# thoglu/jammy_flows

Hardware: AMD Instinct MI355X
Metric: log-prob evals/sec (batch 2^20), e4+s2+e4 / gggg+f+gggg (higher is better)
Workload: dtype f32; 1 GPU; pdf("e4+s2+e4","gggg+f+gggg") log-prob, unconditional pdf with autoregressive conditioning, 1048576 rows in total, row-sharded; batch_per_gpu=1048576, total_rows=1048576, parallelism=rows sharded over 1 GPU(s)

## Files before the change

### jammy_flows_amd/csrc/jf_cond_mchain.h

```cpp
#pragma once
#include <type_traits>

#include "jf_cond_split.h"
#include "jf_manifold.h"
#include "jf_mfma.h"

namespace jf {

constexpr int CM_HMAX = 128, CM_K1MAX = 28, CM_NMAX = 64;

template <typename T, typename CLayer, int NL = JF_MAX_MCHAIN> struct CmArgs {
    const T* in; int64_t in_stride;
    const T* W1; int64_t w1s; const T* b1;
    const T* W2; int64_t w2s; const T* b2;
    int K1, H, N;
    const T* x; int64_t xs;
    const T* ld_in;
    int64_t B;
    int n_layers, dim, tile_stride, scratch, tab;
    int col0[NL];
    CLayer L[NL];
    T* x_out; int64_t xos;
    T* ld_out;
    const T* blp_in; T* blp_out;
    int32_t* status;
};

template <typename T, class Fam, int NT, bool FWD, class Args>
__device__ __forceinline__ void cond_mchain_body(const Args& a, const int block, const int n_blocks, unsigned char* smem_raw) {
    using MF = Mfma16<T>;
    constexpr int MT = 16, KS = 4, NREG = 4, JH = CM_HMAX / MT;
    const int k1p = (a.K1 + KS - 1) / KS * KS, ldk = k1p + 1;
    const int np = (a.N + MT - 1) / MT * MT;
    constexpr int LDW = CM_HMAX + 1;
    T* W1s = reinterpret_cast<T*>(smem_raw);
    T* b1s = W1s + CM_HMAX * ldk;
    T* W2s = b1s + CM_HMAX;
    T* b2s = W2s + np * LDW;
    T* Xs = b2s + np + 8;
    T* tiles = Xs + NT * ldk;
    T* tabs = tiles + NT * a.tile_stride;
    const int tid = threadIdx.x, lane = tid & 63, wave = tid >> 6;
    const int li = lane & 15, lq = lane >> 4;
    const int64_t last = a.B - 1;
    for (int i = tid; i < CM_HMAX * k1p; i += NT) {
        const int r = i / k1p, c = i - r * k1p;
        W1s[r * ldk + c] = (r < a.H && c < a.K1) ? a.W1[(int64_t)r * a.w1s + c] : T(0);
    }
    for (int i = tid; i < CM_HMAX; i += NT) b1s[i] = i < a.H ? a.b1[i] : T(0);
    float w2_inv = 1.f;
    if constexpr (std::is_same<T, float>::value) {
        float amax = 0.f;
        for (int i = tid; i < a.N * a.H; i += NT) {
            const int r = i / a.H, c = i - r * a.H;
            amax = fmaxf(amax, fabsf(a.W2[(int64_t)r * a.w2s + c]));
        }
#pragma unroll
        for (int m = 32; m >= 1; m >>= 1) amax = fmaxf(amax, __shfl_xor(amax, m));
        float* red = reinterpret_cast<float*>(b2s + np);
        if (lane == 0) red[wave] = amax;
        __syncthreads();
        amax = red[0];
        for (int w = 1; w < NT / 64; ++w) amax = fmaxf(amax, red[w]);
        const int e = (amax > 0.f && amax < INFINITY) ? 14 - ilogbf(amax) : 0;
        const float wscale = ldexpf(1.0f, e);
        w2_inv = ldexpf(1.0f, -(e + 14));
        unsigned char* W2p = reinterpret_cast<unsigned char*>(W2s);
        for (int f = tid; f < (np / MT) * CS_KSTEPS * 64; f += NT) {
            const int fl = f & 63, s = (f >> 6) % CS_KSTEPS, ct = (f >> 6) / CS_KSTEPS;
            const int m = fl & 15, q = fl >> 4, col = ct * MT + m;
            f16x8 hi, lo;
#pragma unroll
            for (int i = 0; i < 8; ++i) {
                const int k = 16 * (2 * s + (i >> 2)) + 4 * q + (i & 3);
                const float w = (col < a.N && k < a.H) ? a.W2[(int64_t)col * a.w2s + k] * wscale : 0.f;
                const _Float16 h16 = (_Float16)w;
                hi[i] = h16; lo[i] = (_Float16)(w - (float)h16);
            }
            *reinterpret_cast<f16x8*>(W2p + (size_t)((ct * CS_KSTEPS + s) * 2 + 0) * CS_FRAG + fl * 16) = hi;
            *reinterpret_cast<f16x8*>(W2p + (size_t)((ct * CS_KSTEPS + s) * 2 + 1) * CS_FRAG + fl * 16) = lo;
        }
    } else {
        for (int i = tid; i < np * CM_HMAX; i += NT) {
            const int r = i / CM_HMAX, c = i - r * CM_HMAX;
            W2s[r * LDW + c] = (r < a.N && c < a.H) ? a.W2[(int64_t)r * a.w2s + c] : T(0);
        }
    }
    for (int i = tid; i < np; i += NT) b2s[i] = (i < a.N && a.b2) ? a.b2[i] : T(0);
    for (int64_t row0 = (int64_t)block * NT; row0 < a.B; row0 += (int64_t)n_blocks * NT) {
    __syncthreads();
    for (int i = tid; i < NT * k1p; i += NT) {
        const int r = i / k1p, c = i - r * k1p;
        const int64_t gr = row0 + r;
        Xs[r * ldk + c] = c < a.K1 ? a.in[(gr <= last ? gr : last) * a.in_stride + c] : T(0);
    }
    __syncthreads();

    T* tile = tiles + wave * 64 * a.tile_stride;
    for (int rt = 0; rt < 4; ++rt) {
        T hreg[JH][NREG];
        {
            typename MF::Acc acc[JH];
#pragma unroll
            for (int j = 0; j < JH; ++j)
#pragma unroll
                for (int r = 0; r < NREG; ++r) acc[j][r] = T(0);
            for (int s = 0; s < k1p / KS; ++s) {
                const int kk = s * KS + lq;
                const T xb = Xs[(wave * 64 + rt * MT + li) * ldk + kk];
#pragma unroll
                for (int j = 0; j < JH; ++j) acc[j] = MF::mma(W1s[(j * MT + li) * ldk + kk], xb, acc[j]);
            }
#pragma unroll
            for (int j = 0; j < JH; ++j)
#pragma unroll
                for (int r = 0; r < NREG; ++r) hreg[j][r] = M<T>::tanh_fast(acc[j][r] + b1s[j * MT + MF::row_of(r, lane)]);
        }
        if constexpr (std::is_same<T, float>::value) {
            f16x8 hH[CS_KSTEPS], hL[CS_KSTEPS];
#pragma unroll
            for (int s = 0; s < CS_KSTEPS; ++s) {
                using u32x4 = __attribute__((ext_vector_type(4))) unsigned;
                u32x4 q0, q1;
#pragma unroll
                for (int i = 0; i < 8; i += 2) {
                    const int j = 2 * s + (i >> 2), r = i & 3;
                    unsigned ph, pl;
                    cs_split16(hreg[j][r] * CS_H_SCALE, hreg[j][r + 1] * CS_H_SCALE, ph, pl);
                    q0[i >> 1] = ph; q1[i >> 1] = pl;
                }
                hH[s] = __builtin_bit_cast(f16x8, q0); hL[s] = __builtin_bit_cast(f16x8, q1);
            }
            const unsigned char* W2p = reinterpret_cast<const unsigned char*>(W2s);
            for (int ct = 0; ct < np / MT; ++ct) {
                f32x4 acc = {0.f, 0.f, 0.f, 0.f};
#pragma unroll
                for (int s = 0; s < CS_KSTEPS; ++s) {
                    const f16x8 aH = *reinterpret_cast<const f16x8*>(W2p + (size_t)((ct * CS_KSTEPS + s) * 2 + 0) * CS_FRAG + lane * 16);
                    const f16x8 aL = *reinterpret_cast<const f16x8*>(W2p + (size_t)((ct * CS_KSTEPS + s) * 2 + 1) * CS_FRAG + lane * 16);
                    acc = __builtin_amdgcn_mfma_f32_16x16x32_f16(aL, hH[s], acc, 0, 0, 0);
                    acc = __builtin_amdgcn_mfma_f32_16x16x32_f16(aH, hL[s], acc, 0, 0, 0);
                    acc = __builtin_amdgcn_mfma_f32_16x16x32_f16(aH, hH[s], acc, 0, 0, 0);
                }
#pragma unroll
                for (int v = 0; v < 4; ++v) {
                    const int c = ct * MT + 4 * lq + v;
                    tile[(rt * MT + li) * a.tile_stride + c] = acc[v] * w2_inv + b2s[c];
                }
            }
        } else
        for (int ct = 0; ct < np / MT; ++ct) {
            typename MF::Acc acc;
#pragma unroll
            for (int r = 0; r < NREG; ++r) acc[r] = T(0);
            const T* wrow = W2s + (ct * MT + li) * LDW;
#pragma unroll
            for (int j = 0; j < JH; ++j)
#pragma unroll
                for (int r = 0; r < NREG; ++r) acc = MF::mma(wrow[j * MT + MF::row_of(r, lane)], hreg[j][r], acc);
#pragma unroll
            for (int v = 0; v < NREG; ++v) {
                const int c = ct * MT + MF::row_of(v, lane);
                tile[(rt * MT + li) * a.tile_stride + c] = acc[v] + b2s[c];
            }
        }
    }
    __syncthreads();

    const int64_t row = row0 + tid;
    const bool active = row <= last;
    const int64_t rrow = active ? row : last;
    T x[3] = {T(0), T(0), T(0)};
#pragma unroll
    for (int d = 0; d < Fam::DIM; ++d) if (d < a.dim) x[d] = a.x[rrow * a.xs + d];
    T ld = a.ld_in ? a.ld_in[rrow] : T(0);
    LaneCtx<T> ctx;
    ctx.tab = tabs + tid * (a.tab + a.scratch);
    ctx.corr = ctx.tab + a.tab;
    ctx.bins = nullptr; ctx.bin_i = 0;
    ctx.oob = ctx.nonconv = ctx.nonfinite = false;
    ctx.lane_valid = active;
    const T* prow = tiles + tid * a.tile_stride;
    for (int i = 0; i < a.n_layers; ++i) {
        const int l = FWD ? i : a.n_layers - 1 - i;
        Fam::template apply<T, FWD>(a.L[l], prow + a.col0[l], x, ld, ctx);
    }
    bool bad = !M<T>::finite(ld);
#pragma unroll
    for (int d = 0; d < Fam::DIM; ++d) bad = bad || !M<T>::finite(x[d]);
    if (active) {
#pragma unroll
        for (int d = 0; d < Fam::DIM; ++d) if (d < a.dim) a.x_out[row * a.xos + d] = x[d];
        a.ld_out[row] = ld;
        if (a.blp_out) {
            T s = a.blp_in ? a.blp_in[row] : T(0);
#pragma unroll
            for (int d = 0; d < Fam::DIM; ++d) if (d < a.dim) s += T(-0.5) * x[d] * x[d] - M<T>::HALF_LN_2PI;
            a.blp_out[row] = s;
        }
    }
    status_add(a.status, JF_STATUS_NONFINITE, active && (bad || ctx.nonfinite));
    status_add(a.status, JF_STATUS_OUT_OF_RANGE, active && ctx.oob);
    status_add(a.status, JF_STATUS_NONCONVERGED, active && ctx.nonconv);
    }
}

}
```

### jammy_flows_amd/csrc/jf_manifold.h

```cpp
#pragma once
#include "jf_sphere.h"
#include "jf_spline.h"

namespace jf {

constexpr int JF_CORR_SCRATCH = 81;

template <typename T> struct LaneCtx {
    T* tab;
    T* corr;
    int64_t* bins;
    int bin_i;
    bool oob, nonconv, nonfinite;
    bool lane_valid;
    bool tab_built = false;
    __device__ __forceinline__ void put_bin(int b) {
        if (bins) bins[bin_i] = (int64_t)b;
        ++bin_i;
    }
};

template <typename T> __device__ __forceinline__ SplineDev<T> to_dev(const jf_spline_opts& s) {
    SplineDev<T> o;
    o.nb = s.num_bins; o.smooth = s.smooth; o.fix_first = s.fix_first; o.fix_second = s.fix_second; o.independent = s.independent;
    o.fix_bd = s.fix_bd; o.n_w = s.n_w; o.n_h = s.n_h; o.n_d = s.n_d;
    o.fix_bd_value = (T)s.fix_bd_value; o.min_w = (T)s.min_w; o.min_h = (T)s.min_h; o.min_d = (T)s.min_d; o.ratio = (T)s.ratio;
    return o;
}
__host__ __device__ inline int spline_row_len(const jf_spline_opts& s) { return s.n_w + s.n_h + s.n_d; }

__host__ inline bool sane_hh(int hh) { return hh >= JF_ROT_QUATERNION && hh <= 64; }
__host__ inline bool sane_spline(const jf_spline_opts& s) {
    return s.num_bins >= 1 && s.num_bins <= JF_SPLINE_CAP && s.n_w >= 0 && s.n_w <= 4 * JF_SPLINE_CAP && s.n_h >= 0 &&
           s.n_h <= 4 * JF_SPLINE_CAP && s.n_d >= 0 && s.n_d <= 4 * JF_SPLINE_CAP;
}

template <class Fam, class = void> struct fam_tab_words { static int of(const typename Fam::CLayer&) { return JF_SPLINE_TAB; } };
template <class Fam> struct fam_tab_words<Fam, std::void_t<decltype(&Fam::tab_words)>> { static int of(const typename Fam::CLayer& L) { return Fam::tab_words(L); } };

template <typename T> __device__ __forceinline__ T r_core(const jf_r_layer& L, const T* __restrict__ p, T x, T& ld, LaneCtx<T>& c, bool inverse) {
    x = x > T(1) ? T(1) : (x < T(-1) ? T(-1) : x);
    bool oob;
    const SplineDev<T> o = to_dev<T>(L.sp);
    const SplineOut<T> r = spline_interval<T>(p, o, c.tab, x, inverse, (T)L.lo, (T)L.hi, oob, c.tab_built);
    c.oob = c.oob || oob;
    c.put_bin(r.bin);
    ld += r.lad;
    return r.y > T(1) ? T(1) : (r.y < T(-1) ? T(-1) : r.y);
}
struct RFam {
    using CLayer = jf_r_layer;
    static constexpr int DIM = 1;
    static constexpr bool HAS_BUILD = true;
    template <typename T> static __device__ __forceinline__ void build(const CLayer& L, const T* __restrict__ p, T* __restrict__ tab) {
        spline_interval_build<T>(p, to_dev<T>(L.sp), tab, (T)L.lo, (T)L.hi);
    }
    static __host__ bool sane(const CLayer& L) { return sane_spline(L.sp); }
    static __host__ int row_len(const CLayer& L) { return spline_row_len(L.sp); }
    static __host__ int n_bins(const CLayer&) { return 1; }
    static __host__ bool needs_tab(const CLayer&) { return true; }
    static __host__ int tab_words(const CLayer& L) { return spline_tab_words(L.sp.num_bins); }
    template <typename T, bool FWD> static __device__ __forceinline__ void apply(const CLayer& L, const T* __restrict__ p, T (&x)[3], T& ld, LaneCtx<T>& c) {
        if constexpr (FWD) {
            if (L.first) x[0] = real_line_to_interval<T>(x[0], (T)L.lo, (T)L.hi, ld);
            x[0] = r_core<T>(L, p, x[0], ld, c, false);
        } else {
            x[0] = r_core<T>(L, p, x[0], ld, c, true);
            if (L.first) x[0] = interval_to_real_line<T>(x[0], (T)L.lo, (T)L.hi, ld);
        }
    }
};

template <typename T> __device__ __forceinline__ T s1_rotate(const T* __restrict__ vs, int hh, T phi, bool transpose) {
    T e[3];
    s1_to_eucl<T>(phi, e);
    rotate_embed<T, 2>(vs, hh, e, transpose);
    return eucl_to_s1<T>(e);
}

template <typename T> __device__ __forceinline__ void s2_rotate(const T* __restrict__ vs, int hh, T (&x)[3], T& ld, bool transpose) {
    T e[3];
    s2_to_eucl<T>(x[0], x[1], e, ld);
    rotate_embed<T, 3>(vs, hh, e, transpose);
// ... 228 lines not shown
        }
    }
    static __host__ bool sane(const CLayer& L) {
        if (!sane_hh(L.hh_iter) || L.n_vertical < 0 || L.n_vertical > JF_MAX_NESTED || L.n_circular < 0 || L.n_circular > JF_MAX_NESTED) return false;
        if (L.corr_hidden < 0 || L.corr_hidden > 65536 || L.corr_rank < 0 || L.corr_rank > 65536) return false;
        for (int i = 0; i < L.n_vertical; ++i) if (!sane_spline(L.vertical[i].sp)) return false;
        for (int i = 0; i < L.n_circular; ++i) if (!sane_spline(L.circular[i].sp) || !sane_hh(L.circular[i].hh_iter)) return false;
        return true;
    }
    static __host__ int row_len(const CLayer& L) {
        int n = rot_len(L.hh_iter, 3) + n_kappa(L);
        for (int i = 0; i < L.n_vertical; ++i) n += spline_row_len(L.vertical[i].sp);
        if (L.correlated) return n + corr_len(L);
        for (int i = 0; i < L.n_circular; ++i) n += spline_row_len(L.circular[i].sp);
        return n;
    }
    static __host__ int n_bins(const CLayer& L) { return L.n_vertical + L.n_circular; }
    static __host__ bool needs_tab(const CLayer& L) { return L.n_vertical + L.n_circular > 0; }
    static __host__ int tab_words(const CLayer& L) {
        int w = 1;
        for (int i = 0; i < L.n_vertical && i < JF_MAX_NESTED; ++i) { const int t = spline_tab_words(L.vertical[i].sp.num_bins); w = t > w ? t : w; }
        for (int i = 0; i < L.n_circular && i < JF_MAX_NESTED; ++i) { const int t = spline_tab_words(L.circular[i].sp.num_bins); w = t > w ? t : w; }
        return w;
    }
    static __host__ int scratch(const CLayer& L) { return L.correlated ? JF_CORR_SCRATCH : 0; }

    template <typename T> static __device__ inline void corr_mlp(const CLayer& L, const T* __restrict__ mp, T z, T* __restrict__ out) {
        const int H = L.corr_hidden, R = L.corr_rank, n = corr_out(L);
        const T* W1 = mp;
        const T* b1 = mp + H;
        const T* s2 = mp + 2 * H;
        if (L.corr_full2) {
            const T* b2 = s2 + n * H;
            for (int i = 0; i < n; ++i) out[i] = b2[i];
            for (int j = 0; j < H; ++j) {
                const T h = M<T>::tanh(W1[j] * z + b1[j]);
                for (int i = 0; i < n; ++i) out[i] += s2[i * H + j] * h;
            }
        } else {
            const T* V = s2 + n * R;
            const T* b2 = V + R * H;
            T* t = out + n;
            for (int r = 0; r < R; ++r) t[r] = T(0);
            for (int j = 0; j < H; ++j) {
                const T h = M<T>::tanh(W1[j] * z + b1[j]);
                for (int r = 0; r < R; ++r) t[r] += V[r * H + j] * h;
            }
            for (int i = 0; i < n; ++i) {
                T acc = T(0);
                for (int r = 0; r < R; ++r) acc += s2[i * R + r] * t[r];
                out[i] = acc + b2[i];
            }
        }
    }

    template <typename T> static __device__ __forceinline__ void inv_head(const CLayer& L, const T* __restrict__ p, T (&x)[3], T& ld, T& ret_out, T& angle_out) {
        const T* fp = p + rot_len(L.hh_iter, 3);
        const T zs = (T)L.z_sign;
        const T kappa = kappa_of<T>(L, p, fp);
        if (L.hh_iter != 0) s2_rotate<T>(p, L.hh_iter, x, ld, true);
        const T prev = M<T>::cos(x[0]);
        ld += M<T>::log(M<T>::sin(safe_angle_pi<T>(x[0])));
        const T e2k = M<T>::exp(T(-2) * kappa);
        const T safe = kappa < T(100) ? M<T>::log(M<T>::expm1(T(2) * kappa)) : T(2) * kappa;
        ld += M<T>::log(T(2) * kappa) + kappa * (zs * prev + T(1)) - safe;
        T ret = zs * ((T(1) + e2k - T(2) * M<T>::exp(kappa * (zs * prev - T(1)))) / (T(-1) + e2k));
        if (kappa < M<T>::KAPPA_ID) ret = prev;
        ret = safe_cos<T>(ret, M<T>::EPS_COS);
        T angle = x[1];
        if (L.extra_rotation) inbetween<T>(ret, angle, ld, true);
        ret_out = ret; angle_out = angle;
    }
    template <typename T> static __device__ __forceinline__ void inv_tail(const CLayer& L, T ret, T angle, T (&x)[3], T& ld) {
        ret = safe_cos<T>(ret, M<T>::EPS_COS);
        const T th = M<T>::acos(ret);
        ld -= M<T>::log(M<T>::sin(safe_angle_pi<T>(th)));
        if (L.first) {
            T pl[3];
            s2_to_plane<T>(th, angle, pl, ld);
            x[0] = pl[0]; x[1] = pl[1];
        } else { x[0] = th; x[1] = angle; }
    }

    template <typename T, bool FWD> static __device__ __forceinline__ void apply(const CLayer& L, const T* __restrict__ p, T (&x)[3], T& ld, LaneCtx<T>& c) {
        const T* fp = p + rot_len(L.hh_iter, 3);
        const T zs = (T)L.z_sign, region = (T)L.identity_region;
        const T kappa = kappa_of<T>(L, p, fp);
        int nv = 0;
        for (int i = 0; i < L.n_vertical; ++i) nv += spline_row_len(L.vertical[i].sp);
        const T* vert = fp + n_kappa(L);
        const T* circ = vert + nv;
        if constexpr (!FWD) {
            T ret, angle;
            inv_head<T>(L, p, x, ld, ret, angle);
            const bool inside = (region == T(0)) || ((ret > T(-1) + region) && (ret < T(1) - region));
            if (L.correlated) {
                if (inside) {
                    const T z_in = ret;
                    int off = nv;
                    for (int i = L.n_vertical - 1; i >= 0; --i) {
                        off -= spline_row_len(L.vertical[i].sp);
                        ret = r_core<T>(L.vertical[i], vert + off, ret, ld, c, true);
                    }
                    corr_mlp<T>(L, vert + nv, z_in, c.corr);
                    int coff = corr_out(L);
                    for (int i = L.n_circular - 1; i >= 0; --i) {
                        coff -= rot_len(L.circular[i].hh_iter, 2) + spline_row_len(L.circular[i].sp);
                        T xx[3] = {angle, T(0), T(0)};
                        OFam::apply<T, false>(L.circular[i], c.corr + coff, xx, ld, c);
                        angle = xx[0];
                    }
                } else {
                    for (int i = 0; i < L.n_vertical + L.n_circular; ++i) c.put_bin(-2);
                }
            } else {
            if (L.n_circular > 0) {
                const T sc = azimuthal_scaling<T>(ret);
                int off = 0;
                for (int i = 0; i < L.n_circular; ++i) off += spline_row_len(L.circular[i].sp);
                for (int i = L.n_circular - 1; i >= 0; --i) {
                    off -= spline_row_len(L.circular[i].sp);
                    if (inside) angle = o_core<T>(L.circular[i], circ + off, angle, ld, c, false, sc);
                    else c.put_bin(-2);
                }
            }
            if (L.n_vertical > 0) {
                int off = nv;
                for (int i = L.n_vertical - 1; i >= 0; --i) {
                    off -= spline_row_len(L.vertical[i].sp);
                    if (inside) ret = r_core<T>(L.vertical[i], vert + off, ret, ld, c, true);
                    else c.put_bin(-2);
                }
            }
            }
            inv_tail<T>(L, ret, angle, x, ld);
        } else {
            if (L.first) {
                T pl[3] = {x[0], x[1], T(0)};
                plane_to_s2<T>(pl, x[0], x[1], ld);
            }
            T prev = M<T>::cos(x[0]);
            ld += M<T>::log(M<T>::sin(safe_angle_pi<T>(x[0])));
            T angle = x[1];
            const bool inside = (region == T(0)) || ((prev > T(-1) + region) && (prev < T(1) - region));
            if (L.correlated) {
                if (inside) {
                    int off = 0;
                    for (int i = 0; i < L.n_vertical; ++i) {
                        prev = r_core<T>(L.vertical[i], vert + off, prev, ld, c, false);
                        off += spline_row_len(L.vertical[i].sp);
                    }
                    corr_mlp<T>(L, vert + nv, prev, c.corr);
                    int coff = 0;
                    for (int i = 0; i < L.n_circular; ++i) {
                        T xx[3] = {angle, T(0), T(0)};
                        OFam::apply<T, true>(L.circular[i], c.corr + coff, xx, ld, c);
                        angle = xx[0];
                        coff += rot_len(L.circular[i].hh_iter, 2) + spline_row_len(L.circular[i].sp);
                    }
                } else {
                    for (int i = 0; i < L.n_vertical + L.n_circular; ++i) c.put_bin(-2);
                }
            } else {
            if (L.n_vertical > 0) {
                int off = 0;
                for (int i = 0; i < L.n_vertical; ++i) {
                    if (inside) prev = r_core<T>(L.vertical[i], vert + off, prev, ld, c, false);
                    else c.put_bin(-2);
                    off += spline_row_len(L.vertical[i].sp);
                }
            }
            if (L.n_circular > 0) {
                const T sc = azimuthal_scaling<T>(prev);
                int off = 0;
                for (int i = 0; i < L.n_circular; ++i) {
                    if (inside) angle = o_core<T>(L.circular[i], circ + off, angle, ld, c, true, sc);
                    else c.put_bin(-2);
                    off += spline_row_len(L.circular[i].sp);
                }
            }
            }
            if (L.extra_rotation) inbetween<T>(prev, angle, ld, false);
            ld -= M<T>::log(kappa * zs * prev + kappa / M<T>::tanh(kappa));
            T ret = zs * (T(1) + (T(1) / kappa) * M<T>::log(T(0.5) * (T(1) + zs * prev) + (T(0.5) - T(0.5) * zs * prev) * M<T>::exp(T(-2) * kappa)));
            if (kappa < M<T>::KAPPA_ID) ret = prev;
            ret = safe_cos<T>(ret, M<T>::EPS_COS);
            x[0] = M<T>::acos(ret);
            ld -= M<T>::log(M<T>::sin(safe_angle_pi<T>(x[0])));
            x[1] = angle;
            if (L.hh_iter != 0) s2_rotate<T>(p, L.hh_iter, x, ld, false);
        }
    }
};

}
```

### jammy_flows_amd/csrc/jf_math.h

```cpp
#pragma once
#include <hip/hip_runtime.h>
#include <math.h>

#include "jf_tanh_table.h"

namespace jf {

template <typename T> struct M;

template <typename T> struct DualTraits { static constexpr bool is_dual = false; using value_type = T; };
template <typename D> struct DualValues;



template <> struct M<float> {
    static constexpr float PI = 3.14159265358979323846f;
    static constexpr float TWO_PI = 6.28318530717958647692f;
    static constexpr float HALF_LN_2PI = 0.91893853320467274178f;
    static constexpr float SQRT2 = 1.41421356237309504880f;
    static constexpr float TINY = 1e-35f;
    static constexpr float EPS_COS = 1e-7f;
    static constexpr float EPS_S1 = 1e-5f;
    static constexpr float KAPPA_ID = 1e-4f;
#ifdef JF_PROBE_ACCURATE_EXP
    static __device__ __forceinline__ float exp_fast(float x) { return expf(x); }
#else
    static __device__ __forceinline__ float exp_fast(float x) { return __expf(x); }
#endif
#ifdef JF_PROBE_ACCURATE_LOG
    static __device__ __forceinline__ float log_fast(float x) { return logf(x); }
#else
    static __device__ __forceinline__ float log_fast(float x) { return 0.69314718056f * __builtin_amdgcn_logf(x); }
#endif
#ifdef JF_PROBE_ACCURATE_RCP
    static __device__ __forceinline__ float sqrt_fast(float x) { return sqrtf(x); }
    static __device__ __forceinline__ float rcp(float x) { return __fdiv_rn(1.0f, x); }
#else
    static __device__ __forceinline__ float sqrt_fast(float x) { return __builtin_amdgcn_sqrtf(x); }
    static __device__ __forceinline__ float rcp(float x) { return __builtin_amdgcn_rcpf(x); }
#endif
    static __device__ __forceinline__ float exp(float x) { return expf(x); }
    static __device__ __forceinline__ float log(float x) { return logf(x); }
    static __device__ __forceinline__ float log1p(float x) { return log1pf(x); }
    static __device__ __forceinline__ float expm1(float x) { return expm1f(x); }
    static __device__ __forceinline__ float sqrt(float x) { return sqrtf(x); }
    static __device__ __forceinline__ float erf(float x) { return erff(x); }
    static __device__ __forceinline__ float erfinv(float x) { return erfinvf(x); }
    static __device__ __forceinline__ float erfcinv(float x) { return erfcinvf(x); }
    static __device__ __forceinline__ float sin(float x) { return sinf(x); }
    static __device__ __forceinline__ float cos(float x) { return cosf(x); }
    static __device__ __forceinline__ float acos(float x) { return acosf(x); }
    static __device__ __forceinline__ float atan2(float y, float x) { return atan2f(y, x); }
    static __device__ __forceinline__ float tanh(float x) { return tanhf(x); }
    static __device__ __forceinline__ float tanh_fast(float x) { return 1.0f - 2.0f * __builtin_amdgcn_rcpf(__expf(2.0f * x) + 1.0f); }
    static __device__ __forceinline__ float abs(float x) { return fabsf(x); }
    static __device__ __forceinline__ float max(float a, float b) { return fmaxf(a, b); }
    static __device__ __forceinline__ float min(float a, float b) { return fminf(a, b); }
    static __device__ __forceinline__ bool finite(float x) { return isfinite(x); }
};

template <> struct M<double> {
    static constexpr double PI = 3.14159265358979323846;
    static constexpr double TWO_PI = 6.28318530717958647692;
    static constexpr double HALF_LN_2PI = 0.91893853320467274178;
    static constexpr double SQRT2 = 1.41421356237309504880;
    static constexpr double TINY = 1e-280;
    static constexpr double EPS_COS = 1e-10;
    static constexpr double EPS_S1 = 1e-8;
    static constexpr double KAPPA_ID = 1e-8;
    static __device__ __forceinline__ double exp_fast(double x) { return ::exp(x); }
    static __device__ __forceinline__ double log_fast(double x) {
        int e = __builtin_amdgcn_frexp_exp(x);
        double m = __builtin_amdgcn_frexp_mant(x);
        const bool low = m < 0.70710678118654752440;
        m = low ? m + m : m;
        e = low ? e - 1 : e;
        const double f = m - 1.0;
        const double s = f * rcp(2.0 + f);
        const double z = s * s, w = z * z;
        const double t1 = w * ::fma(w, ::fma(w, 1.531383769920937332e-01, 2.222219843214978396e-01), 3.999999999940941908e-01);
        const double t2 = z * ::fma(w, ::fma(w, ::fma(w, 1.479819860511658591e-01, 1.818357216161805012e-01), 2.857142874366239149e-01),
                                    6.666666666666735130e-01);
        const double R = t1 + t2, hfsq = 0.5 * f * f, de = (double)e;
        double r = ::fma(de, 6.93147180369123816490e-01, -((hfsq - ::fma(s, hfsq + R, de * 1.90821492927058770002e-10)) - f));
        r = x == 0.0 ? -INFINITY : r;
        return (x > 0.0 && x < INFINITY) || x == 0.0 ? r : (x < 0.0 ? NAN : x);
    }
    static __device__ __forceinline__ double sqrt_fast(double x) { return ::sqrt(x); }
    static __device__ __forceinline__ double rcp(double x) {
        const double r0 = __builtin_amdgcn_rcp(x);
        double r = ::fma(::fma(-x, r0, 1.0), r0, r0);
        r = ::fma(::fma(-x, r, 1.0), r, r);
        return isfinite(r) ? r : r0;
    }
    static __device__ __forceinline__ double exp(double x) { return ::exp(x); }
    static __device__ __forceinline__ double log(double x) { return ::log(x); }
    static __device__ __forceinline__ double log1p(double x) { return ::log1p(x); }
    static __device__ __forceinline__ double expm1(double x) { return ::expm1(x); }
    static __device__ __forceinline__ double sqrt(double x) { return ::sqrt(x); }
    static __device__ __forceinline__ double erf(double x) { return ::erf(x); }
    static __device__ __forceinline__ double erfinv(double x) { return ::erfinv(x); }
    static __device__ __forceinline__ double erfcinv(double x) { return ::erfcinv(x); }
    static __device__ __forceinline__ double sin(double x) { return ::sin(x); }
    static __device__ __forceinline__ double cos(double x) { return ::cos(x); }
    static __device__ __forceinline__ double acos(double x) { return ::acos(x); }
    static __device__ __forceinline__ double atan2(double y, double x) { return ::atan2(y, x); }
    static __device__ __forceinline__ double tanh(double x) { return ::tanh(x); }
    static __device__ __forceinline__ double tanh_fast(double x) {
        const double t = ::exp(-2.0 * ::fabs(x));
        return ::copysign((1.0 - t) * rcp(1.0 + t), x);
    }
    static __device__ __forceinline__ double abs(double x) { return ::fabs(x); }
    static __device__ __forceinline__ double max(double a, double b) { return ::fmax(a, b); }
    static __device__ __forceinline__ double min(double a, double b) { return ::fmin(a, b); }
    static __device__ __forceinline__ bool finite(double x) { return isfinite(x); }
};

__device__ __forceinline__ void tanh_tab_load(double* __restrict__ lds_tab, int tid, int nthreads) {
    for (int i = tid; i < JF_TANH_TAB_N; i += nthreads) lds_tab[i] = JF_TANH_TAB[i];
}
__device__ __forceinline__ double tanh_tab(const double* __restrict__ lds_tab, double x) {
#ifdef JF_PROBE_NO_TANH_TAB
    return M<double>::tanh_fast(x);
// ... 41 lines not shown
```

### jammy_flows_amd/csrc/manifold_kernels.hip

```cpp
#include <type_traits>

#include "jf_expmap.h"
#include "jf_manifold.h"

namespace jf {

constexpr int MC_MAX_PRE = 4;
template <typename T, typename CLayer> struct MChainArgs {
    const T* x; int64_t xs;
    const T* ld_in;
    const T* params; int64_t ps;
    int bcast;
    int64_t B;
    int n_layers;
    int dim;
    int tile_stride;
    int scratch;
    int tab;
    int rows;
    int shared_tab;
    int vec_ok[JF_MAX_MCHAIN];
    int col0[JF_MAX_MCHAIN];
    int ncols[JF_MAX_MCHAIN];
    CLayer L[JF_MAX_MCHAIN];
    T* x_out; int64_t xos;
    T* ld_out;
    const T* blp_in; T* blp_out;
    int64_t* bins; int64_t bins_stride;
    int32_t* status;
    const T* ld_pre[MC_MAX_PRE]; const T* blp_pre[MC_MAX_PRE];
    int n_ld_pre, n_blp_pre;
    T* total;
};

template <class Fam, class = void> struct fam_has_build : std::false_type {};
template <class Fam> struct fam_has_build<Fam, std::void_t<decltype(Fam::HAS_BUILD)>> : std::true_type {};

template <typename T, class Fam, bool FWD>
__global__ void __launch_bounds__(64) mchain_kernel(const MChainArgs<T, typename Fam::CLayer> a) {
    extern __shared__ __align__(16) unsigned char smem_raw[];
    T* tile = reinterpret_cast<T*>(smem_raw);
    const int tid = threadIdx.x;
    const int rows = a.rows;
    const int tile_rows = a.bcast ? 1 : rows;
    const bool lane_in = tid < rows;
    const int slot = lane_in ? tid : 0;
    constexpr bool CAN_SHARE = fam_has_build<Fam>::value;
    const bool shared = CAN_SHARE && a.shared_tab != 0;
    T* tab = tile + tile_rows * a.tile_stride + (shared ? 0 : slot * a.tab);
    const int64_t row0 = (int64_t)blockIdx.x * rows;
    const int64_t row = row0 + tid;
    const bool active = lane_in && row < a.B;
    const int64_t rrow = active ? row : a.B - 1;
    const int valid_rows = (int)((a.B - row0) < rows ? (a.B - row0) : rows);

    T x[3] = {T(0), T(0), T(0)};
#pragma unroll
    for (int d = 0; d < Fam::DIM; ++d) if (d < a.dim) x[d] = a.x[rrow * a.xs + d];
    T ld = a.ld_in ? a.ld_in[rrow] : T(0);
    LaneCtx<T> ctx;
    ctx.tab = tab;
    ctx.corr = tile + tile_rows * a.tile_stride + (shared ? 1 : rows) * a.tab + slot * a.scratch;
    ctx.bins = (a.bins && active) ? a.bins + row * a.bins_stride : nullptr;
    ctx.bin_i = 0;
    ctx.oob = ctx.nonconv = ctx.nonfinite = false;
    ctx.lane_valid = active;

    for (int i = 0; i < a.n_layers; ++i) {
        const int l = FWD ? i : a.n_layers - 1 - i;
        __syncthreads();
        if (a.bcast) {
            for (int j = tid; j < a.ncols[l]; j += 64) tile[j] = a.params[a.col0[l] + j];
        } else {
            stage_rows<T>(tile, a.tile_stride, a.params + row0 * a.ps + a.col0[l], a.ps, a.ncols[l], rows, valid_rows, tid, 64, a.vec_ok[l] != 0);
        }
        __syncthreads();
        const T* prow = tile + (a.bcast ? 0 : slot * a.tile_stride);
        if constexpr (CAN_SHARE) {
            if (shared) {
                if (tid == 0) Fam::template build<T>(a.L[l], prow, tab);
                __syncthreads();
                ctx.tab_built = true;
            }
        }
        if (lane_in) Fam::template apply<T, FWD>(a.L[l], prow, x, ld, ctx);
    }
    bool bad = !M<T>::finite(ld);
#pragma unroll
    for (int d = 0; d < Fam::DIM; ++d) bad = bad || !M<T>::finite(x[d]);
    if (active) {
#pragma unroll
        for (int d = 0; d < Fam::DIM; ++d) if (d < a.dim) a.x_out[row * a.xos + d] = x[d];
        T ldv = ld;
        if (a.n_ld_pre > 0) {
            T t = a.ld_pre[0][row];
            for (int i = 1; i < a.n_ld_pre; ++i) t += a.ld_pre[i][row];
            ldv = t + ld;
        }
        a.ld_out[row] = ldv;
        if (a.blp_out) {
            T s = a.blp_in ? a.blp_in[row] : T(0);
#pragma unroll
            for (int d = 0; d < Fam::DIM; ++d) if (d < a.dim) s += T(-0.5) * x[d] * x[d] - M<T>::HALF_LN_2PI;
            if (a.n_blp_pre > 0) {
                T t = a.blp_pre[0][row];
                for (int i = 1; i < a.n_blp_pre; ++i) t += a.blp_pre[i][row];
                s = t + s;
            }
            a.blp_out[row] = s;
            if (a.total) a.total[row] = s + ldv;
        }
    }
    status_add(a.status, JF_STATUS_NONFINITE, active && (bad || ctx.nonfinite));
    status_add(a.status, JF_STATUS_OUT_OF_RANGE, active && ctx.oob);
    status_add(a.status, JF_STATUS_NONCONVERGED, active && ctx.nonconv);
}

template <typename T, class Fam, bool FWD>
static int mchain(const T* x, int64_t xs, const T* ld_in, const T* params, int64_t ps, int32_t pb, int64_t B, int32_t n_layers,
                  const typename Fam::CLayer* layers, T* x_out, int64_t xos, T* ld_out, const T* blp_in, T* blp_out, int64_t* bins,
                  int64_t bins_stride, int32_t* status, void* stream, const jf_row_list* ld_pre = nullptr, const jf_row_list* blp_pre = nullptr,
                  T* total = nullptr) {
    if (!x || !x_out || !ld_out || !layers || n_layers < 1 || n_layers > JF_MAX_MCHAIN || B < 0) return JF_ERR_BADARG;
    if ((ld_pre || blp_pre || total) && (FWD || !blp_out)) return JF_ERR_BADARG;
    if ((ld_pre && (ld_pre->n < 0 || ld_pre->n > MC_MAX_PRE)) || (blp_pre && (blp_pre->n < 0 || blp_pre->n > MC_MAX_PRE))) return JF_ERR_UNSUPPORTED;
    if (ld_pre) for (int i = 0; i < ld_pre->n; ++i) if (!ld_pre->p[i]) return JF_ERR_BADARG;
    if (blp_pre) for (int i = 0; i < blp_pre->n; ++i) if (!blp_pre->p[i]) return JF_ERR_BADARG;
    if (pb != 1 && pb != B) return JF_ERR_BADARG;
    if (B == 0) return JF_OK;
    MChainArgs<T, typename Fam::CLayer> a{};
    a.x = x; a.xs = xs; a.ld_in = ld_in; a.params = params; a.ps = ps; a.bcast = (pb == 1) ? 1 : 0; a.B = B; a.n_layers = n_layers;
    int col = 0, maxp = 0;
    for (int l = 0; l < n_layers; ++l) {
        if (!Fam::sane(layers[l])) return JF_ERR_BADARG;
        a.L[l] = layers[l];
        const int n = Fam::row_len(layers[l]);
        a.col0[l] = col; a.ncols[l] = n;
        a.vec_ok[l] = (!a.bcast && n > 0 && aligned16<T>(params, ps, col) && (n % Vec16<T>::N == 0)) ? 1 : 0;
        col += n;
        if (n > maxp) maxp = n;
    }
    if (col > 0 && !params) return JF_ERR_BADARG;
    a.tile_stride = padded_stride<T>(maxp > 0 ? maxp : 1);
    a.dim = Fam::DIM;
    if constexpr (std::is_same<Fam, CFam>::value) a.dim = layers[0].kind == 2 ? 2 : 1;
    a.x_out = x_out; a.xos = xos; a.ld_out = ld_out; a.blp_in = blp_in; a.blp_out = blp_out; a.bins = bins; a.bins_stride = bins_stride; a.status = status;
    if (ld_pre) { for (int i = 0; i < ld_pre->n; ++i) a.ld_pre[i] = static_cast<const T*>(ld_pre->p[i]); a.n_ld_pre = ld_pre->n; }
    if (blp_pre) { for (int i = 0; i < blp_pre->n; ++i) a.blp_pre[i] = static_cast<const T*>(blp_pre->p[i]); a.n_blp_pre = blp_pre->n; }
    a.total = total;
    a.scratch = 0;
    if constexpr (std::is_same<Fam, FFam>::value) {
        for (int l = 0; l < n_layers; ++l) {
            if (!layers[l].correlated) continue;
            if (layers[l].corr_hidden < 1 || layers[l].corr_rank < 0 || FFam::corr_out(layers[l]) + layers[l].corr_rank > JF_CORR_SCRATCH - 1)
                return JF_ERR_UNSUPPORTED;
            a.scratch = JF_CORR_SCRATCH;
        }
    }
    a.tab = 0;
    for (int l = 0; l < n_layers; ++l)
        if (Fam::needs_tab(layers[l])) { const int w = fam_tab_words<Fam>::of(layers[l]); a.tab = w > a.tab ? w : a.tab; }
    a.rows = 64;
    a.shared_tab = (fam_has_build<Fam>::value && a.bcast && a.tab > 0) ? 1 : 0;
    size_t lds = 0;
    for (;;) {
        lds = ((size_t)(a.bcast ? 1 : a.rows) * a.tile_stride + (size_t)(a.shared_tab ? 1 : a.rows) * a.tab + (size_t)a.rows * a.scratch) * sizeof(T);
        if (lds <= 160 * 1024 || a.rows == 8) break;
        a.rows >>= 1;
// ... 112 lines not shown
```

Before: 1.657 billion log-prob evals/s.

## Fold tanh prescale into W1, vectorize input staging, add specialized f32 inverse sphere path

Pre-multiplies W1 and b1 by 2/ln2 so the hidden tanh becomes exp2+rcp, and seeds the accumulators with the bias instead of adding it afterwards. It stages input rows per thread in chunks of eight. It also adds a dedicated f32 inverse apply for the sphere family that uses polynomial sincos, hardware sin/cos and rsq, and routes both chain kernels through it. Together these target transcendental and scalar overhead in the MLP and the manifold layers, at some cost in accuracy from the approximate intrinsics and a more complex code path.

```diff
diff --git a/jammy_flows_amd/csrc/jf_cond_mchain.h b/jammy_flows_amd/csrc/jf_cond_mchain.h
--- a/jammy_flows_amd/csrc/jf_cond_mchain.h
+++ b/jammy_flows_amd/csrc/jf_cond_mchain.h
@@ -43,11 +43,19 @@
     const int tid = threadIdx.x, lane = tid & 63, wave = tid >> 6;
     const int li = lane & 15, lq = lane >> 4;
     const int64_t last = a.B - 1;
+    constexpr bool F32 = std::is_same<T, float>::value;
+    constexpr T PRE = F32 ? T(2.8853900817779268) : T(1);
     for (int i = tid; i < CM_HMAX * k1p; i += NT) {
         const int r = i / k1p, c = i - r * k1p;
-        W1s[r * ldk + c] = (r < a.H && c < a.K1) ? a.W1[(int64_t)r * a.w1s + c] : T(0);
-    }
-    for (int i = tid; i < CM_HMAX; i += NT) b1s[i] = i < a.H ? a.b1[i] : T(0);
+        T w = (r < a.H && c < a.K1) ? a.W1[(int64_t)r * a.w1s + c] : T(0);
+        if constexpr (F32) w *= PRE;
+        W1s[r * ldk + c] = w;
+    }
+    for (int i = tid; i < CM_HMAX; i += NT) {
+        T b = i < a.H ? a.b1[i] : T(0);
+        if constexpr (F32) b *= PRE;
+        b1s[i] = b;
+    }
     float w2_inv = 1.f;
     if constexpr (std::is_same<T, float>::value) {
         float amax = 0.f;
@@ -89,48 +97,73 @@
     for (int i = tid; i < np; i += NT) b2s[i] = (i < a.N && a.b2) ? a.b2[i] : T(0);
     for (int64_t row0 = (int64_t)block * NT; row0 < a.B; row0 += (int64_t)n_blocks * NT) {
     __syncthreads();
-    for (int i = tid; i < NT * k1p; i += NT) {
-        const int r = i / k1p, c = i - r * k1p;
-        const int64_t gr = row0 + r;
-        Xs[r * ldk + c] = c < a.K1 ? a.in[(gr <= last ? gr : last) * a.in_stride + c] : T(0);
+    if constexpr (F32) {
+        constexpr int CG = 8;
+        const int64_t gr = row0 + tid;
+        const T* src = a.in + (gr <= last ? gr : last) * a.in_stride;
+        T* xr = Xs + tid * ldk;
+        for (int c0 = 0; c0 < k1p; c0 += CG) {
+            T v[CG];
+#pragma unroll
+            for (int u = 0; u < CG; ++u) v[u] = c0 + u < a.K1 ? src[c0 + u] : T(0);
+#pragma unroll
+            for (int u = 0; u < CG; ++u)
+                if (c0 + u < k1p) xr[c0 + u] = v[u];
+        }
+    } else {
+        for (int i = tid; i < NT * k1p; i += NT) {
+            const int r = i / k1p, c = i - r * k1p;
+            const int64_t gr = row0 + r;
+            Xs[r * ldk + c] = c < a.K1 ? a.in[(gr <= last ? gr : last) * a.in_stride + c] : T(0);
+        }
     }
     __syncthreads();
 
     T* tile = tiles + wave * 64 * a.tile_stride;
+#pragma unroll 1
     for (int rt = 0; rt < 4; ++rt) {
         T hreg[JH][NREG];
+        f16x8 hH[CS_KSTEPS], hL[CS_KSTEPS];
         {
             typename MF::Acc acc[JH];
 #pragma unroll
-            for (int j = 0; j < JH; ++j)
-#pragma unroll
-                for (int r = 0; r < NREG; ++r) acc[j][r] = T(0);
+            for (int j = 0; j < JH; ++j) {
+                if constexpr (F32) acc[j] = *reinterpret_cast<const f32x4*>(b1s + j * MT + 4 * lq);
+                else {
+#pragma unroll
+                    for (int r = 0; r < NREG; ++r) acc[j][r] = T(0);
+                }
+            }
             for (int s = 0; s < k1p / KS; ++s) {
                 const int kk = s * KS + lq;
                 const T xb = Xs[(wave * 64 + rt * MT + li) * ldk + kk];
 #pragma unroll
                 for (int j = 0; j < JH; ++j) acc[j] = MF::mma(W1s[(j * MT + li) * ldk + kk], xb, acc[j]);
             }
-#pragma unroll
-            for (int j = 0; j < JH; ++j)
-#pragma unroll
-                for (int r = 0; r < NREG; ++r) hreg[j][r] = M<T>::tanh_fast(acc[j][r] + b1s[j * MT + MF::row_of(r, lane)]);
-        }
-        if constexpr (std::is_same<T, float>::value) {
-            f16x8 hH[CS_KSTEPS], hL[CS_KSTEPS];
-#pragma unroll
-            for (int s = 0; s < CS_KSTEPS; ++s) {
-                using u32x4 = __attribute__((ext_vector_type(4))) unsigned;
-                u32x4 q0, q1;
-#pragma unroll
-                for (int i = 0; i < 8; i += 2) {
-                    const int j = 2 * s + (i >> 2), r = i & 3;
-                    unsigned ph, pl;
-                    cs_split16(hreg[j][r] * CS_H_SCALE, hreg[j][r + 1] * CS_H_SCALE, ph, pl);
-                    q0[i >> 1] = ph; q1[i >> 1] = pl;
-                }
-                hH[s] = __builtin_bit_cast(f16x8, q0); hL[s] = __builtin_bit_cast(f16x8, q1);
-            }
+            if constexpr (F32) {
+#pragma unroll
+                for (int s = 0; s < CS_KSTEPS; ++s) {
+                    using u32x4 = __attribute__((ext_vector_type(4))) unsigned;
+                    u32x4 q0, q1;
+#pragma unroll
+                    for (int i = 0; i < 8; i += 2) {
+                        const int j = 2 * s + (i >> 2), r = i & 3;
+                        const float t0 = fmaf(-2.0f * CS_H_SCALE, __builtin_amdgcn_rcpf(__builtin_amdgcn_exp2f(acc[j][r]) + 1.0f), CS_H_SCALE);
+                        const float t1 = fmaf(-2.0f * CS_H_SCALE, __builtin_amdgcn_rcpf(__builtin_amdgcn_exp2f(acc[j][r + 1]) + 1.0f), CS_H_SCALE);
+                        unsigned ph, pl;
+                        cs_split16_plain(t0, t1, ph, pl);
+                        q0[i >> 1] = ph; q1[i >> 1] = pl;
+                    }
+                    hH[s] = __builtin_bit_cast(f16x8, q0); hL[s] = __builtin_bit_cast(f16x8, q1);
+                }
+            } else {
+#pragma unroll
+                for (int j = 0; j < JH; ++j)
+#pragma unroll
+                    for (int r = 0; r < NREG; ++r) hreg[j][r] = M<T>::tanh_fast(acc[j][r] + b1s[j * MT + MF::row_of(r, lane)]);
+            }
+        }
+        if constexpr (F32) {
             const unsigned char* W2p = reinterpret_cast<const unsigned char*>(W2s);
             for (int ct = 0; ct < np / MT; ++ct) {
                 f32x4 acc = {0.f, 0.f, 0.f, 0.f};
@@ -167,7 +200,9 @@
     }
     __syncthreads();
 
-    const int64_t row = row0 + tid;
+    int lt = tid;
+    asm volatile("" : "+v"(lt));
+    const int64_t row = row0 + lt;
     const bool active = row <= last;
     const int64_t rrow = active ? row : last;
     T x[3] = {T(0), T(0), T(0)};
@@ -175,15 +210,15 @@
     for (int d = 0; d < Fam::DIM; ++d) if (d < a.dim) x[d] = a.x[rrow * a.xs + d];
     T ld = a.ld_in ? a.ld_in[rrow] : T(0);
     LaneCtx<T> ctx;
-    ctx.tab = tabs + tid * (a.tab + a.scratch);
+    ctx.tab = tabs + lt * (a.tab + a.scratch);
     ctx.corr = ctx.tab + a.tab;
     ctx.bins = nullptr; ctx.bin_i = 0;
     ctx.oob = ctx.nonconv = ctx.nonfinite = false;
     ctx.lane_valid = active;
-    const T* prow = tiles + tid * a.tile_stride;
+    const T* prow = tiles + lt * a.tile_stride;
     for (int i = 0; i < a.n_layers; ++i) {
         const int l = FWD ? i : a.n_layers - 1 - i;
-        Fam::template apply<T, FWD>(a.L[l], prow + a.col0[l], x, ld, ctx);
+        apply_hot<Fam, T, FWD>(a.L[l], prow + a.col0[l], x, ld, ctx);
     }
     bool bad = !M<T>::finite(ld);
 #pragma unroll
diff --git a/jammy_flows_amd/csrc/jf_manifold.h b/jammy_flows_amd/csrc/jf_manifold.h
--- a/jammy_flows_amd/csrc/jf_manifold.h
+++ b/jammy_flows_amd/csrc/jf_manifold.h
@@ -1,4 +1,5 @@
 #pragma once
+#include <type_traits>
 #include "jf_sphere.h"
 #include "jf_spline.h"
 
@@ -393,6 +394,50 @@
         } else { x[0] = th; x[1] = angle; }
     }
 
+    template <typename T> static __device__ __forceinline__ void inv_nested(const CLayer& L, const T* __restrict__ vert, const T* __restrict__ circ, int nv,
+                                                                            T region, T& ret, T& angle, T& ld, LaneCtx<T>& c) {
+        const bool inside = (region == T(0)) || ((ret > T(-1) + region) && (ret < T(1) - region));
+        if (L.correlated) {
+            if (inside) {
+                const T z_in = ret;
+                int off = nv;
+                for (int i = L.n_vertical - 1; i >= 0; --i) {
+                    off -= spline_row_len(L.vertical[i].sp);
+                    ret = r_core<T>(L.vertical[i], vert + off, ret, ld, c, true);
+                }
+                corr_mlp<T>(L, vert + nv, z_in, c.corr);
+                int coff = corr_out(L);
+                for (int i = L.n_circular - 1; i >= 0; --i) {
+                    coff -= rot_len(L.circular[i].hh_iter, 2) + spline_row_len(L.circular[i].sp);
+                    T xx[3] = {angle, T(0), T(0)};
+                    OFam::apply<T, false>(L.circular[i], c.corr + coff, xx, ld, c);
+                    angle = xx[0];
+                }
+            } else {
+                for (int i = 0; i < L.n_vertical + L.n_circular; ++i) c.put_bin(-2);
+            }
+        } else {
+        if (L.n_circular > 0) {
+            const T sc = azimuthal_scaling<T>(ret);
+            int off = 0;
+            for (int i = 0; i < L.n_circular; ++i) off += spline_row_len(L.circular[i].sp);
+            for (int i = L.n_circular - 1; i >= 0; --i) {
+                off -= spline_row_len(L.circular[i].sp);
+                if (inside) angle = o_core<T>(L.circular[i], circ + off, angle, ld, c, false, sc);
+                else c.put_bin(-2);
+            }
+        }
+        if (L.n_vertical > 0) {
+            int off = nv;
+            for (int i = L.n_vertical - 1; i >= 0; --i) {
+                off -= spline_row_len(L.vertical[i].sp);
+                if (inside) ret = r_core<T>(L.vertical[i], vert + off, ret, ld, c, true);
+                else c.put_bin(-2);
+            }
+        }
+        }
+    }
+
     template <typename T, bool FWD> static __device__ __forceinline__ void apply(const CLayer& L, const T* __restrict__ p, T (&x)[3], T& ld, LaneCtx<T>& c) {
         const T* fp = p + rot_len(L.hh_iter, 3);
         const T zs = (T)L.z_sign, region = (T)L.identity_region;
@@ -404,46 +449,7 @@
         if constexpr (!FWD) {
             T ret, angle;
             inv_head<T>(L, p, x, ld, ret, angle);
-            const bool inside = (region == T(0)) || ((ret > T(-1) + region) && (ret < T(1) - region));
-            if (L.correlated) {
-                if (inside) {
-                    const T z_in = ret;
-                    int off = nv;
-                    for (int i = L.n_vertical - 1; i >= 0; --i) {
-                        off -= spline_row_len(L.vertical[i].sp);
-                        ret = r_core<T>(L.vertical[i], vert + off, ret, ld, c, true);
-                    }
-                    corr_mlp<T>(L, vert + nv, z_in, c.corr);
-                    int coff = corr_out(L);
-                    for (int i = L.n_circular - 1; i >= 0; --i) {
-                        coff -= rot_len(L.circular[i].hh_iter, 2) + spline_row_len(L.circular[i].sp);
-                        T xx[3] = {angle, T(0), T(0)};
-                        OFam::apply<T, false>(L.circular[i], c.corr + coff, xx, ld, c);
-                        angle = xx[0];
-                    }
-                } else {
-                    for (int i = 0; i < L.n_vertical + L.n_circular; ++i) c.put_bin(-2);
-                }
-            } else {
-            if (L.n_circular > 0) {
-                const T sc = azimuthal_scaling<T>(ret);
-                int off = 0;
-                for (int i = 0; i < L.n_circular; ++i) off += spline_row_len(L.circular[i].sp);
-                for (int i = L.n_circular - 1; i >= 0; --i) {
-                    off -= spline_row_len(L.circular[i].sp);
-                    if (inside) angle = o_core<T>(L.circular[i], circ + off, angle, ld, c, false, sc);
-                    else c.put_bin(-2);
-                }
-            }
-            if (L.n_vertical > 0) {
-                int off = nv;
-                for (int i = L.n_vertical - 1; i >= 0; --i) {
-                    off -= spline_row_len(L.vertical[i].sp);
-                    if (inside) ret = r_core<T>(L.vertical[i], vert + off, ret, ld, c, true);
-                    else c.put_bin(-2);
-                }
-            }
-            }
+            inv_nested<T>(L, vert, circ, nv, region, ret, angle, ld, c);
             inv_tail<T>(L, ret, angle, x, ld);
         } else {
             if (L.first) {
@@ -502,6 +508,72 @@
             if (L.hh_iter != 0) s2_rotate<T>(p, L.hh_iter, x, ld, false);
         }
     }
+
+    static __device__ __forceinline__ void apply_inv_f32(const CLayer& L, const float* __restrict__ p, float (&x)[3], float& ld, LaneCtx<float>& c) {
+        using T = float;
+        const T* fp = p + rot_len(L.hh_iter, 3);
+        const T zs = (T)L.z_sign, region = (T)L.identity_region;
+        const T kappa = kappa_of<T>(L, p, fp);
+        int nv = 0;
+        for (int i = 0; i < L.n_vertical; ++i) nv += spline_row_len(L.vertical[i].sp);
+        const T* vert = fp + n_kappa(L);
+        const T* circ = vert + nv;
+        const bool need_angle = L.extra_rotation || L.correlated || L.n_circular > 0 || !L.first;
+        T st, prev;
+        M<T>::sincos_polar(safe_angle_pi<T>(x[0]), st, prev);
+        ld += M<T>::log_fast(st);
+        T angle = x[1], cphi = T(1), sphi = T(0);
+        bool have_cs = false;
+        if (L.hh_iter != 0) {
+            T sp, cp;
+            M<T>::sincos_turn(x[1], sp, cp);
+            T e[3] = {st * cp, st * sp, prev};
+            if (L.hh_iter > 0) {
+                for (int i = 0; i < L.hh_iter; ++i) {
+                    const T* v = p + 3 * i;
+                    const T f = T(2) * (v[0] * e[0] + v[1] * e[1] + v[2] * e[2]) * M<T>::rcp(v[0] * v[0] + v[1] * v[1] + v[2] * v[2]);
+                    e[0] -= f * v[0]; e[1] -= f * v[1]; e[2] -= f * v[2];
+                }
+            } else rotate_embed<T, 3>(p, L.hh_iter, e, true);
+            const T rho2 = e[0] * e[0] + e[1] * e[1];
+            const T q = e[2] * M<T>::rsq(rho2 + e[2] * e[2]);
+            prev = q > T(1) ? T(1) : (q < T(-1) ? T(-1) : q);
+            if (need_angle) angle = azimuth<T>(e[0], e[1]);
+            else {
+                const bool pole = !(rho2 > T(1e-30));
+                const T ir = M<T>::rsq(pole ? T(1) : rho2);
+                cphi = pole ? T(1) : e[0] * ir; sphi = pole ? T(0) : e[1] * ir;
+                have_cs = true;
+            }
+        }
+        const T e2k = M<T>::exp(T(-2) * kappa);
+        const T safe = kappa < T(100) ? M<T>::log(M<T>::expm1(T(2) * kappa)) : T(2) * kappa;
+        ld += M<T>::log(T(2) * kappa) + kappa * (zs * prev + T(1)) - safe;
+        T ret = zs * ((T(1) + e2k - T(2) * M<T>::exp(kappa * (zs * prev - T(1)))) * M<T>::rcp(T(-1) + e2k));
+        if (kappa < M<T>::KAPPA_ID) ret = prev;
+        ret = safe_cos<T>(ret, M<T>::EPS_COS);
+        if (L.extra_rotation) inbetween<T>(ret, angle, ld, true);
+        inv_nested<T>(L, vert, circ, nv, region, ret, angle, ld, c);
+        ret = safe_cos<T>(ret, M<T>::EPS_COS);
+        if (L.first) {
+            const T om = T(1) - safe_cos<T>(ret, T(1e-6));
+            const T lh = M<T>::log(om * T(0.5));
+            ld -= lh + T(0.69314718055994531);
+            const T r = M<T>::sqrt_fast(T(-2) * lh);
+            if (!have_cs) M<T>::sincos_turn(angle, sphi, cphi);
+            x[0] = r * cphi; x[1] = r * sphi;
+        } else {
+            x[0] = M<T>::acos(ret);
+            ld -= T(0.5) * M<T>::log_fast((T(1) - ret) * (T(1) + ret));
+            x[1] = angle;
+        }
+    }
 };
 
-}
+template <class Fam, typename T, bool FWD>
+__device__ __forceinline__ void apply_hot(const typename Fam::CLayer& L, const T* __restrict__ p, T (&x)[3], T& ld, LaneCtx<T>& c) {
+    if constexpr (std::is_same<Fam, FFam>::value && std::is_same<T, float>::value && !FWD) FFam::apply_inv_f32(L, p, x, ld, c);
+    else Fam::template apply<T, FWD>(L, p, x, ld, c);
+}
+
+}
diff --git a/jammy_flows_amd/csrc/jf_math.h b/jammy_flows_amd/csrc/jf_math.h
--- a/jammy_flows_amd/csrc/jf_math.h
+++ b/jammy_flows_amd/csrc/jf_math.h
@@ -39,6 +39,28 @@
     static __device__ __forceinline__ float sqrt_fast(float x) { return __builtin_amdgcn_sqrtf(x); }
     static __device__ __forceinline__ float rcp(float x) { return __builtin_amdgcn_rcpf(x); }
 #endif
+    static __device__ __forceinline__ float rsq(float x) { return __builtin_amdgcn_rsqf(x); }
+    static __device__ __forceinline__ void sincos_turn(float x, float& s, float& c) {
+        const float t = x * 0.15915494309189535f;
+        s = __builtin_amdgcn_sinf(t); c = __builtin_amdgcn_cosf(t);
+    }
+    static __device__ __forceinline__ void sincos_polar(float th, float& s, float& c) {
+        const bool up = th > 1.57079632679489662f;
+        const float u = up ? (3.14159274101257324f - th) + -8.74227765734758577e-8f : th;
+        const float z = u * u;
+        float ps = fmaf(z, -2.50521083854417188e-8f, 2.75573192239858907e-6f);
+        ps = fmaf(z, ps, -1.98412698412698413e-4f);
+        ps = fmaf(z, ps, 8.33333333333333333e-3f);
+        ps = fmaf(z, ps, -1.66666666666666667e-1f);
+        s = fmaf(u * z, ps, u);
+        float pc = fmaf(z, 2.08767569878680990e-9f, -2.75573192239858907e-7f);
+        pc = fmaf(z, pc, 2.48015873015873016e-5f);
+        pc = fmaf(z, pc, -1.38888888888888889e-3f);
+        pc = fmaf(z, pc, 4.16666666666666667e-2f);
+        pc = fmaf(z, pc, -0.5f);
+        pc = fmaf(z, pc, 1.0f);
+        c = up ? -pc : pc;
+    }
     static __device__ __forceinline__ float exp(float x) { return expf(x); }
     static __device__ __forceinline__ float log(float x) { return logf(x); }
     static __device__ __forceinline__ float log1p(float x) { return log1pf(x); }
diff --git a/jammy_flows_amd/csrc/manifold_kernels.hip b/jammy_flows_amd/csrc/manifold_kernels.hip
--- a/jammy_flows_amd/csrc/manifold_kernels.hip
+++ b/jammy_flows_amd/csrc/manifold_kernels.hip
@@ -83,7 +83,7 @@
                 ctx.tab_built = true;
             }
         }
-        if (lane_in) Fam::template apply<T, FWD>(a.L[l], prow, x, ld, ctx);
+        if (lane_in) apply_hot<Fam, T, FWD>(a.L[l], prow, x, ld, ctx);
     }
     bool bad = !M<T>::finite(ld);
 #pragma unroll
```

After: 1.714 billion log-prob evals/s (median of 6 runs). 3.4% higher.
